# gercap/gr-ofdm_tools

Hardware: AMD Instinct MI355X
Metric: IQ Msamples/s Welch-PSD (4096-pt, 50% ovlp) (higher is better)
Workload: dtype f32; 1 GPU; C2: 2^28-sample complex64 stream, 4096-pt Hann Welch, 50% overlap, detrend constant, density; nfft=4096, noverlap=2048, window=hann, samples_per_gpu=268435456, segments_per_gpu=131071, parallelism=single GPU

## Files before the change

### gr-ofdm_tools_amd/csrc/abi_state.h

```cpp
#pragma once
#include "../../include/ofdm_tools_hip.h"
#include "oth_internal.h"
#include "abi_barrier.h"
#include "abi_mem.h"

#include <algorithm>
#include <cmath>
#include <cstdio>
#include <cstdlib>
#include <cstring>
#include <map>
#include <memory>
#include <mutex>
#include <new>
#include <string>
#include <vector>

using namespace oth;

struct oth_ctx {
    int device = 0;
    hipStream_t stream = nullptr;
    bool own_stream = false;
    int cu_count = 256;
    std::string err;
    std::string name;
    bool timing = false;
    std::vector<std::pair<Event, Event>> events;
    std::vector<std::pair<Event, Event>> free_events;
    double total_ms = 0.0;
    uint64_t launches = 0;
    std::map<int, DevBuf<float2>> twiddles;
    DevBuf<float> sink;
    DevBuf<double> acc4;
    DevBuf<unsigned> queue;
    unsigned *done_count = nullptr;
    std::recursive_mutex mu;
    bool queue_clean = false;
    int queue_used = 0;
    DevBuf<unsigned char> scratch;
    std::vector<int> bounds_host;
    DevBuf<int> d_bounds;
    PinnedBuf<int> h_bounds;
    Event bounds_ev;
    ~oth_ctx() {
        if (own_stream) hipStreamDestroy(stream);
    }
};

struct AnyTables {
    AnyShape sh{};
    const float2 *tw = nullptr;
    DevBuf<float2> chirp;
    DevBuf<float2> midtab;
    DevBuf<float2> ws;
    DevBuf<float4> mean;
};

struct oth_plan {
    oth_ctx *ctx = nullptr;
    int nfft = 0, nperseg = 0, noverlap = 0, step = 0, detrend = 0, scaling = 0, fftshift = 0, trim = 0;
    int db = 0, kernel = OTH_KERNEL_AUTO, sched = OTH_SCHED_DYNAMIC;
    double fs = 1.0, scale = 1.0;
    DevBuf<float> d_win;
    const float2 *d_tw = nullptr;
    DevBuf<float4> d_fd;
    DevBuf<float4> d_fd1x;
    DevBuf<float2> d_pilot;
    bool fast_detrend = false;
    bool rect_window = false;
    bool compl_window = false;
    DevBuf<float> d_partial;
    DevBuf<float> d_reduce;
    DevBuf<float> d_out;
    static constexpr int kOutRing = 4;
    PinnedBuf<float> h_out;
    PinnedBuf<unsigned> h_seq;
    uint64_t out_ticket[kOutRing] = {0, 0, 0, 0};
    uint64_t out_nseg[kOutRing] = {0, 0, 0, 0};
    uint64_t next_out_ticket = 1;
    bool pilot_launch = false;
    std::string last_recipe;
    DevBuf<float2> d_stage;
    DevBuf<float> d_sum;
    DevBuf<float> d_wpm;
    uint64_t nseg_total = 0;
    size_t carry = 0;
    DevBuf<float2> d_stream;
    std::string tune_variant;
    int tune_sched = -1, tune_chunk = 0, tune_tail = 0;
    PinnedBuf<char> h_ring[4];
    Event h_ring_ev[4];
    unsigned h_ring_next = 0;
    AnyTables any;
    std::mutex exec_mu;
    int hostwait = 0;
    int average = OTH_AVERAGE_MEAN;
    DevBuf<float> d_rows;
    DevBuf<float> d_med;
    DevBuf<unsigned> d_msel;
    AnyTables rows_any;
    long long bias_nseg = 0;
    double bias = 1.0;
    int ntapers = 0;
    DevBuf<float> d_tapers;
    DevBuf<float> d_coef;
};

struct oth_chain {
    oth_ctx *ctx = nullptr;
    int nfft = 0, fftshift = 0, epilogue = 0, keep_n = 1, count = 1;
    DevBuf<float> d_win;
    const float2 *d_tw = nullptr;
    DevBuf<float2> d_buf;
    size_t leftover = 0;
    DevBuf<float> d_rows;
    int do_iir = 0, do_peak = 0;
    float alpha = 0.f, kdb = 0.f;
    DevBuf<float> d_iir, d_peak;
// ... 182 lines not shown
```

### gr-ofdm_tools_amd/csrc/abi_welch.hip

```cpp
#include "abi_state.h"

#include <sched.h>
#include <time.h>

namespace {
bool window_spectrum(const std::vector<float> &w, int n, int band, std::vector<double> &re, std::vector<double> &im) {
    re.assign(n, 0.0);
    im.assign(n, 0.0);
    double s2 = 0.0;
    for (int i = 0; i < n; ++i) {
        re[i] = (double)w[i];
        s2 += (double)w[i] * (double)w[i];
    }
    host_fft_pow2(re, im);
    for (int k = band; k < n - band; ++k)
        if (re[k] * re[k] + im[k] * im[k] > 1e-10 * s2) return false;
    return true;
}

bool window_spectrum_table(const std::vector<float> &w, std::vector<float> &fd) {
    std::vector<double> re, im;
    if (!window_spectrum(w, 4096, 256, re, im)) return false;
    fd.resize(4 * 256);
    for (int t = 0; t < 256; ++t) {
// ... 5 lines not shown
    }
    return true;
}

bool window_spectrum_table_seg(const std::vector<float> &w, int n, std::vector<float> &fd) {
    const int R = n / 256, Q = 16 / R;
    std::vector<double> re, im;
    if (!window_spectrum(w, n, 256, re, im)) return false;
    fd.assign((size_t)4 * (n / 16) * Q, 0.f);
    for (int t = 0; t < n / 16; ++t) {
        const int k0 = t / R, j = t % R;
        for (int m = 0; m < Q; ++m) {
            const int lo = k0 + 16 * (j + R * m), hi = lo + 256 * (R - 1);
            float *o = &fd[4 * ((size_t)Q * t + m)];
            o[0] = (float)re[lo];
            o[1] = (float)im[lo];
            o[2] = (float)re[hi];
            o[3] = (float)im[hi];
        }
    }
    return true;
}

bool window_spectrum_table_16k(const std::vector<float> &w, int n, std::vector<float> &fd) {
    const int F = n / 4096;
    std::vector<double> re, im;
    if (!window_spectrum(w, n, 256 * F, re, im)) return false;
    fd.assign((size_t)4 * 256 * F, 0.f);
    for (int tid = 0; tid < 256 * F; ++tid) {
        const int kp = tid >> 8, k0 = (tid >> 4) & 15, k1 = tid & 15;
        const int lo = kp + F * (k0 + 16 * k1), hi = kp + F * (k0 + 16 * k1 + 3840);
        fd[4 * tid] = (float)re[lo];
        fd[4 * tid + 1] = (float)im[lo];
        fd[4 * tid + 2] = (float)re[hi];
        fd[4 * tid + 3] = (float)im[hi];
    }
    return true;
}

bool window_spectrum_table_1x(const std::vector<float> &w, int n, std::vector<float> &fd) {
    std::vector<double> re, im;
    if (!window_spectrum(w, n, 16, re, im)) return false;
    fd.assign((size_t)4 * (n / 16), 0.f);
    for (int k0 = 0; k0 < 16; ++k0) {
        const int lo = n == 16384 ? 64 * k0 : 64 * (k0 >> 1) + 32 * (k0 & 1);
        const int hi = n == 16384 ? 64 * k0 + 63 : 64 * (k0 >> 1) + 32 * (k0 & 1) + 31;
        fd[4 * lo] = (float)re[k0];
        fd[4 * lo + 1] = (float)im[k0];
        const int kh = n - 16 + k0;
        fd[4 * hi + 2] = (float)(-im[kh]);
        fd[4 * hi + 3] = (float)re[kh];
    }
    return true;
}

bool window_is_complementary(const std::vector<float> &w, int n) {
    for (int i = 0; i < n / 2; ++i)
        if (!(std::fabs((double)w[i] + (double)w[i + n / 2] - 1.0) <= 1.1920928955078125e-07)) return false;
    return true;
}

int segments(const oth_plan *p, size_t nsamples, long long *nseg) {
    if (nsamples < (size_t)p->nperseg) return OTH_ERR_INVALID;
    *nseg = (long long)((nsamples - (size_t)p->noverlap) / (size_t)p->step);
    return OTH_OK;
}

int run_average(oth_plan *p, const float2 *x, const float2 *y, size_t nsamples, int nstreams, size_t stride,
                long long *nseg_out, int *W_out, int *layout_out) {
    oth_ctx *c = p->ctx;
    long long nseg = 0;
    if (segments(p, nsamples, &nseg) != OTH_OK)
        return fail(c, OTH_ERR_INVALID, "input shorter than nperseg");
    const bool csd = (y != nullptr);
    if (p->ntapers) {
        if (csd) return refuse_mtm(p, "the cross spectrum", "the taper loop holds one channel");
        if (int rc = mtm_run(p, x, nseg, nstreams, stride, W_out)) return rc;
        *nseg_out = nseg;
        *layout_out = 0;
        return OTH_OK;
    }
    LaunchRecipe r;
    const char *why = "";
    if (int rrc = resolve_recipe(shape_of(p), csd, nseg, nstreams, c->cu_count, runtime_bpc, &r, &why))
        return fail(c, rrc, why);
    p->last_recipe = recipe_text(r, p->nfft);
    int rc = p->d_partial.ensure(c, sizeof(float) * (size_t)nstreams * r.W * r.nch * p->nfft);
    {
        const int groups = std::max(kReduceGroups, finalize_row_groups(p->nfft, r.W, r.nch));
        if (!rc) rc = p->d_reduce.ensure(c, sizeof(float) * (size_t)nstreams * groups * r.nch * p->nfft);
    }
    if (rc) return rc;
    const float4 *fd_tab = r.form == 2 ? (r.use_fd1x ? p->d_fd1x.get() : p->d_fd.get()) : nullptr;
    const float2 *pilot = nullptr;
    if (r.pilot == 1) {
        rc = p->d_pilot.ensure(c, sizeof(float2) * 2 * kPilotProbes * (size_t)nstreams);
        if (rc) return rc;
        HIPCHK(c, launch_pilot_mean(x, csd ? y : nullptr, stride, p->nperseg, p->step, nseg, nstreams, p->d_pilot.get(), c->stream));
        pilot = p->d_pilot.get();
    }
    unsigned *queue = nullptr;
    if (r.tickets) {
        queue = c->queue.get();
        if (!c->queue_clean) HIPCHK(c, hipMemsetAsync(c->queue.get(), 0, sizeof(unsigned) * 64, c->stream));
        c->queue_clean = false;
        c->queue_used = nstreams;
// ... 18 lines not shown
                         1.0f, 0, p->tune_variant == "anycov");
            if (rc) return rc;
        }
    } else if (r.kern == RK_SEG || r.kern == RK_SEGWS || r.kern == RK_SEGPAD) {
        SegArgs g{};
        g.x = x;
        g.stream_stride = stride;
        g.nstreams = nstreams;
        g.win = p->d_win.get();
        g.tw = p->d_tw;
        g.first = 0;
        g.step = p->step;
        g.nseg = nseg;
        g.detrend = p->detrend;
        g.chain = 0;
        g.partial = p->d_partial.get();
        g.wg_per_stream = r.W;
        g.sched = r.sched;
        g.chunk = r.chunk;
        g.tail_chunk = r.tail_chunk;
        g.nbig = r.nbig;
        g.queue = queue;
        g.fd = fd_tab;
        g.pilot = pilot;
        Timed tm(c);
        switch (r.kern) {
            case RK_SEGPAD: HIPCHK(c, launch_seg_padded(p->nfft, p->nperseg, g, r.seg_kind, c->stream)); break;
            case RK_SEGWS: HIPCHK(c, launch_segws(p->nfft, g, r.seg_det, c->stream)); break;
            default: HIPCHK(c, launch_seg(p->nfft, g, r.seg_kind, r.seg_wps4, c->stream)); break;
        }
    } else {
        WelchArgs a;
        a.x = x;
        a.y = y;
        a.win = p->d_win.get();
        a.tw = p->d_tw;
        a.partial = p->d_partial.get();
        a.nseg = nseg;
        a.stream_stride = stride;
        a.nperseg = p->nperseg;
        a.step = p->step;
        a.detrend = p->detrend;
        a.wg_per_stream = r.W;
        a.nstreams = nstreams;
        a.sched = r.sched;
        a.chunk = r.chunk;
        a.tail_chunk = r.tail_chunk;
        a.nbig = r.nbig;
        a.queue = queue;
        a.fd = fd_tab;
        a.pilot = pilot;
        a.pilot_inline = r.pilot == 2 ? 1 : 0;
        a.compl_win = p->compl_window && p->tune_variant != "wsgen" ? 1 : 0;
        Timed tm(c);
        switch (r.kern) {
            case RK_W4096: HIPCHK(c, r.variant->launch(a, c->stream)); break;
            case RK_CSD4096WS: HIPCHK(c, launch_csd_tuned4096ws(a, c->stream)); break;
            case RK_CSD4096: HIPCHK(c, launch_csd_tuned4096(a, c->stream)); break;
            case RK_W16K1X_HALF:
                HIPCHK(c, r.half_ws ? launch_welch_tuned8kws(a, c->stream) : launch_welch_tuned16k1x_half(p->nfft, a, c->stream));
                break;
            case RK_W16K1X: HIPCHK(c, launch_welch_tuned16k1x(p->nfft, a, r.x1_window, r.x1_plain, c->stream)); break;
            case RK_W16K: HIPCHK(c, launch_welch_tuned16k(p->nfft, a, c->stream)); break;
            default: HIPCHK(c, launch_welch_generic(p->nfft, a, c->stream)); break;
        }
    }
    *nseg_out = nseg;
    *W_out = r.W;
    *layout_out = r.layout;
    return OTH_OK;
}

int finalize_and_rearm(oth_ctx *c, FinalizeArgs &f, int nstreams) {
    f.queue_reset = nullptr;
    f.queue_n = 0;
    if (!c->queue_clean && c->queue_used > 0) {
        f.queue_reset = c->queue.get();
        f.queue_n = c->queue_used;
    }
    HIPCHK(c, launch_finalize(f, nstreams, c->stream));
    if (f.queue_reset) {
        c->queue_clean = true;
        c->queue_used = 0;
    }
    return OTH_OK;
}

FinalizeArgs finalize_args(const oth_plan *p, int W, int layout, int nch) {
    FinalizeArgs f{};
    f.partial = p->d_partial.get();
    f.scratch = p->d_reduce.get();
    f.W = W;
    f.nfft = p->nfft;
    f.nch = nch;
    f.layout = layout;
    f.l1 = p->any.sh.L1, f.l2 = p->any.sh.L2;
    return f;
}

double median_bias(long long n) {
    double b = 1.0;
    for (long long i = 1; i <= (n - 1) / 2; ++i) b += 1.0 / (double)(2 * i + 1) - 1.0 / (double)(2 * i);
    return b;
}

int refuse_median(oth_plan *p, const char *what) {
// ... 96 lines not shown
    if (use_device(c)) return OTH_ERR_HIP;
    std::unique_ptr<oth_plan> p(new (std::nothrow) oth_plan());
    if (!p) return fail(c, OTH_ERR_NOMEM, "host allocation failed");
    p->ctx = c;
    p->nfft = nfft;
    p->nperseg = nperseg;
    p->noverlap = noverlap;
    p->step = nperseg - noverlap;
    p->fast_detrend = detrend == OTH_DETREND_CONSTANT_FAST;
    p->detrend = detrend != OTH_DETREND_NONE ? OTH_DETREND_CONSTANT : OTH_DETREND_NONE;
    p->scaling = scaling;
    p->fs = fs;
    p->fftshift = fftshift != 0;
    p->trim = trim_bins;
    if (const char *e = getenv("OTH_HOSTWAIT")) p->hostwait = !strcmp(e, "sync") ? 1 : 0;
    *out = std::move(p);
    return OTH_OK;
}
}

extern "C" {

int oth_welch_plan(oth_ctx *c, int nfft, int nperseg, int noverlap, const float *window, int detrend, int scaling,
                   double fs, int fftshift, int trim_bins, oth_plan **out) {
    OTH_TRY
    CtxGuard guard_(c);
    if (!c || !out) return fail(c, OTH_ERR_INVALID, "ctx/out is NULL");
    *out = nullptr;
    std::unique_ptr<oth_plan> p;
    if (int rc = plan_begin(c, nfft, nperseg, noverlap, detrend, scaling, fs, fftshift, trim_bins, &p)) return rc;
    const bool any_route = !generic_supported(nfft);
    const bool det = p->detrend == OTH_DETREND_CONSTANT;
    if (const char *e = getenv("OTH_W4096_VARIANT")) p->tune_variant = e;
    if (const char *e = getenv("OTH_W4096_SCHED")) p->tune_sched = atoi(e);
    if (const char *e = getenv("OTH_W4096_CHUNK")) p->tune_chunk = atoi(e);
    if (const char *e = getenv("OTH_W4096_TAIL")) p->tune_tail = atoi(e);
    if (const char *e = getenv("OTH_PILOT_LAUNCH")) p->pilot_launch = atoi(e) != 0;
    std::vector<float> w(nfft, 0.f);
    double s1 = 0.0, s2 = 0.0;
    p->rect_window = true;
    for (int i = 0; i < nperseg; ++i) {
        w[i] = window ? window[i] : 1.0f;
        if (w[i] != 1.0f) p->rect_window = false;
        s1 += (double)w[i];
        s2 += (double)w[i] * (double)w[i];
    }
    switch (scaling) {
        case OTH_SCALE_DENSITY: p->scale = 1.0 / (fs * s2); break;
        case OTH_SCALE_OVER_N2: p->scale = 1.0 / ((double)nfft * (double)nfft); break;
        case OTH_SCALE_SPECTRUM: p->scale = 1.0 / (s1 * s1); break;
        default: p->scale = 1.0;
    }
    p->compl_window = nfft == 4096 && nperseg == 4096 && window_is_complementary(w, nfft);
    std::vector<float> fd, fd1x, wpm;
    const bool have_fd = det && ((nfft == 4096 && nperseg == 4096 && window_spectrum_table(w, fd)) ||
                                 (nfft == 2048 && nperseg == 2048 && window_spectrum_table_seg(w, nfft, fd)) ||
                                 ((nfft == 8192 || nfft == 16384) && nperseg == nfft && window_spectrum_table_16k(w, nfft, fd)));
    const bool have_fd1x = det && (nfft == 16384 || nfft == 8192) && nperseg == nfft && window_spectrum_table_1x(w, nfft, fd1x);
    if (any_route && nfft == 65536 && nperseg == 65536) {
        wpm.resize(65536);
        for (int n = 0; n < 32768; ++n) {
            wpm[n] = (float)((double)w[n] + (double)w[n + 32768]);
            wpm[32768 + n] = (float)((double)w[n] - (double)w[n + 32768]);
        }
    }
    if (int rc = any_route ? any_tables_init(c, nfft, &p->any) : get_twiddles(c, nfft, &p->d_tw)) return rc;
    hipError_t e = p->d_win.upload(c, w.data(), sizeof(float) * nfft);
    if (e == hipSuccess) e = p->d_sum.alloc(sizeof(float) * nfft);
    if (e == hipSuccess) e = hipMemsetAsync(p->d_sum.get(), 0, sizeof(float) * nfft, c->stream);
    if (e == hipSuccess && have_fd) e = p->d_fd.upload(c, fd.data(), sizeof(float) * fd.size());
    if (e == hipSuccess && have_fd1x) e = p->d_fd1x.upload(c, fd1x.data(), sizeof(float) * fd1x.size());
    if (e == hipSuccess && !wpm.empty()) e = p->d_wpm.upload(c, wpm.data(), sizeof(float) * wpm.size());
    const hipError_t es = hipStreamSynchronize(c->stream);
    if (e == hipSuccess) e = es;
    if (e != hipSuccess) return fail(c, OTH_ERR_HIP, std::string("plan setup: ") + hipGetErrorString(e));
    *out = p.release();
    return OTH_OK;
    OTH_CATCH(c)
}

int oth_plan_destroy(oth_plan *p) {
    OTH_TRY
    CtxGuard guard_(p ? p->ctx : nullptr);
    if (!p) return OTH_OK;
    oth_ctx *c = p->ctx;
    hipSetDevice(c->device);
    hipStreamSynchronize(c->stream);
    delete p;
    return OTH_OK;
    OTH_CATCH((p ? p->ctx : nullptr))
}

int oth_plan_set_output_db(oth_plan *p, int enable) {
    OTH_TRY
    CtxGuard guard_(p ? p->ctx : nullptr);
    if (!p) return fail(nullptr, OTH_ERR_INVALID, "plan is NULL");
    p->db = enable != 0;
    return OTH_OK;
    OTH_CATCH((p ? p->ctx : nullptr))
}

int oth_plan_set_kernel(oth_plan *p, int which) {
    OTH_TRY
    CtxGuard guard_(p ? p->ctx : nullptr);
    if (!p) return fail(nullptr, OTH_ERR_INVALID, "plan is NULL");
    if (which < OTH_KERNEL_AUTO || which > OTH_KERNEL_TUNED) return fail(p->ctx, OTH_ERR_INVALID, "unknown kernel id");
    if (p->ntapers && which == OTH_KERNEL_TUNED) return refuse_mtm(p, "OTH_KERNEL_TUNED", "no tuned kernel carries the taper loop");
    p->kernel = which;
    return OTH_OK;
    OTH_CATCH((p ? p->ctx : nullptr))
}

int oth_plan_set_schedule(oth_plan *p, int which) {
    OTH_TRY
    CtxGuard guard_(p ? p->ctx : nullptr);
    if (!p) return fail(nullptr, OTH_ERR_INVALID, "plan is NULL");
    if (which < OTH_SCHED_CONTIGUOUS || which > OTH_SCHED_DYNAMIC) return fail(p->ctx, OTH_ERR_INVALID, "unknown schedule");
    p->sched = which;
    return OTH_OK;
    OTH_CATCH((p ? p->ctx : nullptr))
}

int oth_plan_set_tuning(oth_plan *p, const char *variant, int sched, int chunk, int tail_chunk) {
// ... 567 lines not shown
```

### gr-ofdm_tools_amd/csrc/fft4096.hip.h

```cpp
#pragma once
#include "fft_lds.hip.h"
#include "oth_internal.h"

static_assert(oth::kPilotProbes == 8, "load_pilot() (fft_lds.hip.h) adds eight probe means");

namespace oth {
namespace {

constexpr int T4 = 256;
constexpr int RS = 272;
constexpr int LDS_X = 16 * RS;
constexpr int LDS_RED = 16;
constexpr size_t LDS_BYTES = (LDS_X + LDS_RED) * sizeof(float2);

constexpr float C1 = 0.92387953251128674f;
constexpr float S1 = 0.38268343236508977f;
constexpr float RH = 0.70710678118654752f;

__device__ __forceinline__ float2 mul_w1(float2 a) { return make_float2(fmaf(a.x, C1, a.y * S1), fmaf(a.y, C1, -a.x * S1)); }
__device__ __forceinline__ float2 mul_w2(float2 a) { return make_float2((a.x + a.y) * RH, (a.y - a.x) * RH); }
__device__ __forceinline__ float2 mul_w3(float2 a) { return make_float2(fmaf(a.x, S1, a.y * C1), fmaf(a.y, S1, -a.x * C1)); }
__device__ __forceinline__ float2 mul_w4(float2 a) { return make_float2(a.y, -a.x); }
__device__ __forceinline__ float2 mul_w6(float2 a) { return make_float2((a.y - a.x) * RH, -(a.x + a.y) * RH); }
__device__ __forceinline__ float2 mul_w9(float2 a) { return make_float2(-fmaf(a.x, C1, a.y * S1), fmaf(a.x, S1, -a.y * C1)); }
// ... 75 lines not shown
        v[1] = cadd(e1, o1);
        v[5] = csub(e1, o1);
        v[2] = cadd(e2, o2);
        v[6] = csub(e2, o2);
        v[3] = cadd(e3, o3);
        v[7] = csub(e3, o3);
        return;
    }
    const float2 p1 = make_float2(v[3].x + v[3].y, v[3].y - v[3].x);
    const float2 p3 = make_float2(v[7].y - v[7].x, -v[7].x - v[7].y);
    v[0] = cadd(e0, o0);
    v[4] = csub(e0, o0);
    v[1] = make_float2(fmaf(RH, p1.x, e1.x), fmaf(RH, p1.y, e1.y));
    v[5] = make_float2(fmaf(-RH, p1.x, e1.x), fmaf(-RH, p1.y, e1.y));
    v[2] = cadd(e2, o2);
    v[6] = csub(e2, o2);
    v[3] = make_float2(fmaf(RH, p3.x, e3.x), fmaf(RH, p3.y, e3.y));
    v[7] = make_float2(fmaf(-RH, p3.x, e3.x), fmaf(-RH, p3.y, e3.y));
}

template <int STRIDE, class F, class M>
__device__ __forceinline__ void dft16_from_lds(float2 (&v)[16], const float2 *base, F issued, M mid) {
    const unsigned addr = (unsigned)(unsigned long long)base;
    double r[16];
#define OTH_LDS_READ(i) asm volatile("ds_read_b64 %0, %1 offset:%2" : "=v"(r[i]) : "v"(addr), "n"(8 * STRIDE * (i)))
    OTH_LDS_READ(0); OTH_LDS_READ(4); OTH_LDS_READ(8); OTH_LDS_READ(12);
    OTH_LDS_READ(1); OTH_LDS_READ(5); OTH_LDS_READ(9); OTH_LDS_READ(13);
    OTH_LDS_READ(2); OTH_LDS_READ(6); OTH_LDS_READ(10); OTH_LDS_READ(14);
    OTH_LDS_READ(3); OTH_LDS_READ(7); OTH_LDS_READ(11); OTH_LDS_READ(15);
#undef OTH_LDS_READ
    issued();
#define OTH_LDS_WAIT(n, a, dep) \
    asm volatile("s_waitcnt lgkmcnt(" #n ")" : "+v"(r[a]), "+v"(r[a + 4]), "+v"(r[a + 8]), "+v"(r[a + 12]), "+v"(dep))
    float dep = 0.f;
#pragma unroll
    for (int a0 = 0; a0 < 4; ++a0) {
        if (a0 == 0) OTH_LDS_WAIT(12, 0, dep);
        else if (a0 == 1) OTH_LDS_WAIT(8, 1, v[0].x);
        else if (a0 == 2) OTH_LDS_WAIT(4, 2, v[1].x);
        else OTH_LDS_WAIT(0, 3, v[2].x);
#pragma unroll
        for (int j = 0; j < 4; ++j) v[a0 + 4 * j] = __builtin_bit_cast(float2, r[a0 + 4 * j]);
        dft4<false>(v[a0], v[a0 + 4], v[a0 + 8], v[a0 + 12]);
    }
#undef OTH_LDS_WAIT
    mid();
    dft16_layer2(v);
}
template <int STRIDE, class F>
__device__ __forceinline__ void dft16_from_lds(float2 (&v)[16], const float2 *base, F issued) {
    dft16_from_lds<STRIDE>(v, base, issued, [] {});
}

__device__ __forceinline__ float2 load_once(const float2 *p) {
    typedef float f2 __attribute__((ext_vector_type(2)));
    const f2 r = __builtin_nontemporal_load(reinterpret_cast<const f2 *>(p));
    return make_float2(r.x, r.y);
}

__device__ __forceinline__ void load_win(float &dst, unsigned lane_off, const char *row) {
    asm volatile("global_load_dword %0, %1, %2" : "=v"(dst) : "v"(lane_off), "s"(row) : "memory");
}

__device__ __forceinline__ long long chunk_count(const WelchArgs &p) {
    const long long rest = p.nseg - p.nbig * p.chunk;
    return p.nbig + (rest + p.tail_chunk - 1) / p.tail_chunk;
}
__device__ __forceinline__ void chunk_range(const WelchArgs &p, long long c, long long &sb, long long &se) {
    if (c < p.nbig) {
        sb = c * p.chunk;
        se = sb + p.chunk;
    } else {
        sb = p.nbig * p.chunk + (c - p.nbig) * p.tail_chunk;
        se = sb + p.tail_chunk < p.nseg ? sb + p.tail_chunk : p.nseg;
    }
}

template <class I> __device__ __forceinline__ I chunk_count_of(I nseg, I nbig, int chunk, int tail_chunk) {
    const I rest = nseg - nbig * chunk;
    return nbig + (rest + tail_chunk - 1) / tail_chunk;
}
template <class I> __device__ __forceinline__ void chunk_range_of(I nseg, I nbig, int chunk, int tail_chunk, I c, I &sb, I &se) {
    if (c < nbig) {
        sb = c * chunk;
        se = sb + chunk;
    } else {
        sb = nbig * chunk + (c - nbig) * tail_chunk;
        se = sb + tail_chunk < nseg ? sb + tail_chunk : nseg;
    }
}

__device__ __forceinline__ void prio_latency() { __builtin_amdgcn_s_setprio(2); }
__device__ __forceinline__ void prio_compute() { __builtin_amdgcn_s_setprio(0); }

__device__ __forceinline__ void lds_barrier() { asm volatile("s_waitcnt lgkmcnt(0)\n\ts_barrier" ::: "memory"); }

template <int STRIDE>
__device__ __forceinline__ void scatter_pow16(const float2 (&v)[16], float2 *out, float2 p1, float2 p4) {
    float2 wj[4], wi[4];
    wj[1] = p1;
    wi[1] = p4;
    asm volatile("" : "+v"(wj[1].x), "+v"(wj[1].y), "+v"(wi[1].x), "+v"(wi[1].y));
    wj[2] = cmul(wj[1], wj[1]);
    wj[3] = cmul(wj[2], wj[1]);
    wi[2] = cmul(wi[1], wi[1]);
    wi[3] = cmul(wi[2], wi[1]);
// ... 111 lines not shown
```

### gr-ofdm_tools_amd/csrc/oth_internal.h

```cpp
#pragma once
#include <hip/hip_runtime.h>
#include <stdint.h>
#include <stddef.h>

namespace oth {

constexpr int kPilotProbes = 8;

struct WelchArgs {
    const float2 *x;
    const float2 *y;
    const float *win;
    const float2 *tw;
    float *partial;
    long long nseg;
    size_t stream_stride;
    int nperseg;
    int step;
    int detrend;
    int wg_per_stream;
    int nstreams;
    int sched;
    int chunk;
    int tail_chunk;
    long long nbig;
    unsigned *queue;
    const float4 *fd;
    const float2 *pilot;
    int pilot_inline;
    int compl_win;
};

struct SegArgs {
    const float2 *x;
    size_t stream_stride;
    int nstreams;
    const float *win;
    const float2 *tw;
    const float4 *fd;
    const float2 *pilot;
    long long first;
    long long step;
    long long nseg;
    int detrend;
    int chain;
    float *partial;
    int acc_mode;
    long long acc_end;
    float l2;
    float *rows;
    long long store_from;
    int epilogue;
    float scale;
    int fftshift;
    int wg_per_stream;
    int sched;
    int chunk;
    int tail_chunk;
    long long nbig;
    unsigned *queue;
};

struct PgramArgs {
    const float2 *x;
    const float *win;
    const float2 *tw;
    float *rows;
    long long first_vec;
    long long nrows;
    int keep_n;
    int fftshift;
    int epilogue;
    float scale;
};

constexpr int kReduceGroups = 16;
inline int finalize_row_groups(int nfft, int W, int nch) {
    if (nch != 1 || nfft > 1024 || (nfft % 256) != 0 || W < 1024) return 0;
    return 65536 / nfft;
}

struct FinalizeArgs {
    const float *partial;
// ... 229 lines not shown
```

### gr-ofdm_tools_amd/csrc/welch4096ws.hip

```cpp

#include <type_traits>
#include "fft4096.hip.h"

namespace oth {
namespace {

constexpr int TWS = 512;
constexpr int WS_RED = 32;
constexpr int WS_CTRL = 16;
constexpr size_t WS_WIN_BYTES = 256 * 2 * sizeof(float4);
constexpr size_t WS_LDS_BYTES = (2 * LDS_X + WS_RED) * sizeof(float2) + WS_CTRL * sizeof(int) + WS_WIN_BYTES;

constexpr int WS_PAL = 2, WS_PAC = 0, WS_PAS = WS_PAL, WS_PBL = 2;
constexpr int WS_PBC = 1;

enum { ITEM_STOP = 0, ITEM_DATA = 1, ITEM_BUBBLE = 2 };

#ifndef OTH_WS_COMPL_POWERS
#define OTH_WS_COMPL_POWERS 13
#endif
constexpr int WS_COMPL_POWERS = OTH_WS_COMPL_POWERS;

template <bool DETREND, bool PILOT, bool COMPL>
__device__ __forceinline__ void welch4096ws_body(const WelchArgs &p) {
    static_assert(DETREND || !PILOT, "the pilot belongs to the detrend");
    extern __shared__ __attribute__((aligned(16))) unsigned char smem[];
    float2 *img = reinterpret_cast<float2 *>(smem);
    float2 *red = img + 2 * LDS_X;
    int *ctrl = reinterpret_cast<int *>(red + WS_RED);

    const int tid = threadIdx.x;
    const bool producer = tid < 256;
    const int t = tid & 255;
    const int hi = t >> 4, lo = t & 15;
    const int wave = t >> 6;
    const int wg = blockIdx.x, W = p.wg_per_stream, stream = blockIdx.y;
    const float2 *xb = p.x + (size_t)stream * p.stream_stride;
    const int sched = p.sched;
    const long long nchunks = sched ? chunk_count(p) : 1;

    const int w1 = hi * 17 + lo, r1 = hi * RS + lo, w2 = hi * RS + lo, r2 = hi * RS + lo * 17;

    if (producer) {
        float win[COMPL ? 1 : 8];
        float4 *wl = reinterpret_cast<float4 *>(ctrl + WS_CTRL) + t;
        constexpr int WROW = COMPL ? 0 : 8;
        if constexpr (!COMPL) {
#pragma unroll
            for (int a = 0; a < 8; ++a) win[a] = p.win[256 * a + t];
        }
        wl[0] = make_float4(p.win[256 * WROW + t], p.win[256 * (WROW + 1) + t], p.win[256 * (WROW + 2) + t], p.win[256 * (WROW + 3) + t]);
        wl[256] = make_float4(p.win[256 * (WROW + 4) + t], p.win[256 * (WROW + 5) + t], p.win[256 * (WROW + 6) + t],
                              p.win[256 * (WROW + 7) + t]);
        const float2 b1 = p.tw[t], b2 = p.tw[2 * t], b3 = p.tw[3 * t], b4 = p.tw[4 * t], b8 = p.tw[8 * t],
                     b12 = p.tw[(12 * t) & 4095];
        float2 bm[WS_COMPL_POWERS - 6 > 0 && COMPL ? WS_COMPL_POWERS - 6 : 1];
        if constexpr (COMPL) {
#pragma unroll
            for (int k = 0; k < WS_COMPL_POWERS - 6; ++k) bm[k] = p.tw[((5 + k + k / 3) * t) & 4095];
        }
        float2 kw[8], nxt[8];
        float2 prev_new = make_float2(0.f, 0.f);
        float2 pv = make_float2(0.f, 0.f);
        if (PILOT && !p.pilot_inline) pv = load_pilot(p.pilot, stream);
        int it = 0;
        unsigned ticket = 0;
        using std::false_type;
        using std::true_type;
        using mid = std::integral_constant<int, 0>;
        using head = std::integral_constant<int, 1>;
        using none = std::integral_constant<int, 2>;

        auto uni = [](int v) { return __builtin_amdgcn_readfirstlane(v); };
// ... 100 lines not shown
            }
            sb = uni((int)((p.nseg * wg) / W));
            se = uni((int)((p.nseg * (wg + 1)) / W));
            return sb < se;
        };
        bool have = open_chunk(sched ? wg : 0);
        if (have) load_chunk_head(sb);
        if (PILOT && p.pilot_inline) {
            const bool own = sched == 0 && have;
            const PilotProbes probes = inline_pilot_load(own ? xb + (size_t)sb * 2048 : xb, own ? (long long)(se - sb) : p.nseg, 2048, t);
            inline_pilot_store(probes, t, img + LDS_X);
            lds_barrier();
            pv = inline_pilot_value(img + LDS_X);
        }
        while (have) {
            const int n = se - sb;
            int ncur = 0;
            if (n >= 2) {
                item(true_type{}, mid{}, sb, 0, n == 2);
                int s = sb + 1;
                if (s < se - 1) item(false_type{}, mid{}, s++, 0, true);
                for (; s + 1 < se - 1; s += 2) {
                    item(false_type{}, mid{}, s, 0, false);
                    item(false_type{}, mid{}, s + 1, 0, false);
                }
                if (s < se - 1) item(false_type{}, mid{}, s, 0, false);
                ncur = (sched == 1) ? cur + W : W + uni(ctrl[4]);
                int nsb = 0, nse = 0;
                const bool have_next = sched && ncur < nchunks;
                if (have_next) {
                    range(ncur, nsb, nse);
                    item(false_type{}, head{}, se - 1, nsb, false);
                    cur = ncur;
                    sb = nsb;
                    se = nse;
                    continue;
                }
                item(false_type{}, none{}, se - 1, 0, false);
                break;
            }
            item(true_type{}, none{}, sb, 0, true);
            if (sched == 0) break;
            if (sched == 2) {
                step_end(ITEM_BUBBLE);
                ncur = W + uni(ctrl[4]);
            } else {
                ncur = cur + W;
            }
            have = open_chunk(ncur);
            if (have) load_chunk_head(sb);
        }
        step_end(ITEM_STOP);
    } else {
        float2 tw2[16];
#pragma unroll
        for (int k = 1; k < 16; ++k) tw2[k] = p.tw[16 * lo * k];
        float4 fw = make_float4(0.f, 0.f, 0.f, 0.f);
        if (DETREND) fw = p.fd[t];
        float acc[16];
#pragma unroll
        for (int k = 0; k < 16; ++k) acc[k] = 0.f;
        float2 v[16];
        float2 mean = make_float2(0.f, 0.f);
        asm volatile("s_waitcnt vmcnt(0)"
                     : "+v"(tw2[1].x), "+v"(tw2[1].y), "+v"(tw2[2].x), "+v"(tw2[2].y), "+v"(tw2[3].x), "+v"(tw2[3].y), "+v"(tw2[4].x),
                       "+v"(tw2[4].y), "+v"(tw2[5].x), "+v"(tw2[5].y), "+v"(tw2[6].x), "+v"(tw2[6].y), "+v"(tw2[7].x), "+v"(tw2[7].y));
        asm volatile("" : "+v"(tw2[8].x), "+v"(tw2[8].y), "+v"(tw2[9].x), "+v"(tw2[9].y), "+v"(tw2[10].x), "+v"(tw2[10].y),
                          "+v"(tw2[11].x), "+v"(tw2[11].y), "+v"(tw2[12].x), "+v"(tw2[12].y), "+v"(tw2[13].x), "+v"(tw2[13].y));
        asm volatile("" : "+v"(tw2[14].x), "+v"(tw2[14].y), "+v"(tw2[15].x), "+v"(tw2[15].y), "+v"(fw.x), "+v"(fw.y), "+v"(fw.z),
                          "+v"(fw.w));
        int it = 0;
        auto next_item = [&]() -> int {
            __builtin_amdgcn_s_setprio(WS_PBL);
            lds_barrier();
            const int q = it & 1;
            const float2 *lq = img + q * LDS_X;
            const int kind = ctrl[q];
            const float2 h0 = red[q * 8], h1 = red[q * 8 + 1], h2 = red[q * 8 + 2], h3 = red[q * 8 + 3];
            dft16_from_lds<17>(v, lq + r1, [] { __builtin_amdgcn_s_setprio(WS_PBC); });
            if (DETREND) {
                const float2 tot = cadd(cadd(h0, h1), cadd(h2, h3));
                mean = make_float2(tot.x * (1.0f / 4096.0f), tot.y * (1.0f / 4096.0f));
            }
            ++it;
            return kind;
        };
        if (PILOT && p.pilot_inline) lds_barrier();
        int item = next_item();
        for (;;) {
            while (item == ITEM_BUBBLE) item = next_item();
            if (item == ITEM_STOP) break;
            float2 *lx = img + ((it & 1) ^ 1) * LDS_X;
            __builtin_amdgcn_s_setprio(WS_PBL);
            lx[w2] = v[r16(0)];
#pragma unroll
            for (int k1 = 1; k1 < 16; ++k1) lx[w2 + k1 * 17] = cmul(v[r16(k1)], tw2[k1]);
            wave_lds_sync();
            dft16_from_lds<1>(v, lx + r2, [] { __builtin_amdgcn_s_setprio(WS_PBC); });
            if (DETREND) {
                v[r16(0)] = make_float2(v[r16(0)].x - (mean.x * fw.x - mean.y * fw.y),
                                        v[r16(0)].y - (mean.x * fw.y + mean.y * fw.x));
                v[r16(15)] = make_float2(v[r16(15)].x - (mean.x * fw.z - mean.y * fw.w),
                                         v[r16(15)].y - (mean.x * fw.w + mean.y * fw.z));
            }
#pragma unroll
            for (int k2 = 0; k2 < 16; ++k2) {
                const float2 X = v[r16(k2)];
                acc[k2] = fmaf(X.x, X.x, fmaf(X.y, X.y, acc[k2]));
            }
            item = next_item();
        }
        float *dst = p.partial + ((size_t)stream * W + wg) * 4096;
#pragma unroll
        for (int k2 = 0; k2 < 16; ++k2) dst[256 * k2 + t] = acc[k2];
    }
}

template <bool DETREND, bool PILOT = false>
__global__ __launch_bounds__(TWS, 4) void welch4096ws_kernel(WelchArgs p) {
    welch4096ws_body<DETREND, PILOT, false>(p);
}
template <bool DETREND, bool PILOT = false>
__global__ __launch_bounds__(TWS, 4) void welch4096ws_compl_kernel(WelchArgs p) {
    welch4096ws_body<DETREND, PILOT, true>(p);
}

}

int tuned4096_blocks_per_cu_ws() {
    static int cached = 0;
    if (cached) return cached;
    int n = 0;
    if (hipOccupancyMaxActiveBlocksPerMultiprocessor(&n, welch4096ws_kernel<true, false>, TWS, WS_LDS_BYTES) != hipSuccess || n < 1)
        n = 1;
    return cached = n;
}

hipError_t launch_welch_tuned4096_ws(const WelchArgs &a, hipStream_t s) {
    const dim3 grid(a.wg_per_stream, a.nstreams);
    static bool armed[64] = {};
    int dev = 0;
    if (hipGetDevice(&dev) != hipSuccess || dev < 0 || dev >= 64) dev = 63, armed[63] = false;
    bool &big_lds = armed[dev];
    if (!big_lds) {
        hipError_t e = hipSuccess;
        for (const void *fn : {reinterpret_cast<const void *>(welch4096ws_kernel<true, true>),
                               reinterpret_cast<const void *>(welch4096ws_kernel<true, false>),
                               reinterpret_cast<const void *>(welch4096ws_kernel<false, false>),
                               reinterpret_cast<const void *>(welch4096ws_compl_kernel<true, true>),
                               reinterpret_cast<const void *>(welch4096ws_compl_kernel<true, false>),
                               reinterpret_cast<const void *>(welch4096ws_compl_kernel<false, false>)})
            if (e == hipSuccess) e = hipFuncSetAttribute(fn, hipFuncAttributeMaxDynamicSharedMemorySize, (int)WS_LDS_BYTES);
        if (e != hipSuccess) return e;
        big_lds = true;
    }
    const bool pilot = a.detrend && (a.pilot || a.pilot_inline);
    if (a.compl_win) {
        if (pilot) hipLaunchKernelGGL((welch4096ws_compl_kernel<true, true>), grid, dim3(TWS), WS_LDS_BYTES, s, a);
        else if (a.detrend) hipLaunchKernelGGL((welch4096ws_compl_kernel<true, false>), grid, dim3(TWS), WS_LDS_BYTES, s, a);
        else hipLaunchKernelGGL((welch4096ws_compl_kernel<false, false>), grid, dim3(TWS), WS_LDS_BYTES, s, a);
    } else if (pilot)
        hipLaunchKernelGGL((welch4096ws_kernel<true, true>), grid, dim3(TWS), WS_LDS_BYTES, s, a);
    else if (a.detrend)
        hipLaunchKernelGGL((welch4096ws_kernel<true, false>), grid, dim3(TWS), WS_LDS_BYTES, s, a);
    else
        hipLaunchKernelGGL((welch4096ws_kernel<false, false>), grid, dim3(TWS), WS_LDS_BYTES, s, a);
    return hipGetLastError();
}

}
```

Before: 455,600 Msamples/s.

## Use tangent-factored twiddles in 4096-pt Welch FFT second pass

Replaces the complex twiddle multiplies between the two radix-16 passes with tangent-form multiplies (one FMA per component), deferring the cosine factors into a scaled radix-16 DFT whose constants come from a per-thread precomputed table. The goal is to cut VALU work in the FFT inner loop of the work-stealing 4096 kernel. It adds 33 per-thread table registers (more VGPR pressure) and a host-side table build, and tan-based factoring can lose accuracy near small cosines, which the code handles by clamping.

```diff
diff --git a/gr-ofdm_tools_amd/csrc/abi_state.h b/gr-ofdm_tools_amd/csrc/abi_state.h
--- a/gr-ofdm_tools_amd/csrc/abi_state.h
+++ b/gr-ofdm_tools_amd/csrc/abi_state.h
@@ -65,6 +65,7 @@
     DevBuf<float> d_win;
     const float2 *d_tw = nullptr;
     DevBuf<float4> d_fd;
+    DevBuf<float> d_tantw;
     DevBuf<float4> d_fd1x;
     DevBuf<float2> d_pilot;
     bool fast_detrend = false;
diff --git a/gr-ofdm_tools_amd/csrc/abi_welch.hip b/gr-ofdm_tools_amd/csrc/abi_welch.hip
--- a/gr-ofdm_tools_amd/csrc/abi_welch.hip
+++ b/gr-ofdm_tools_amd/csrc/abi_welch.hip
@@ -81,6 +81,34 @@
         fd[4 * hi + 3] = (float)re[kh];
     }
     return true;
+}
+
+void tangent_twiddle_table(std::vector<float> &tab) {
+    const double kClamp = 1.0 / 1073741824.0, c1 = std::cos(M_PI / 8.0), rh = std::sqrt(0.5);
+    auto split = [&](int m, double &c, double &t) {
+        const double a = -2.0 * M_PI * (double)(m & 255) / 256.0;
+        c = std::cos(a);
+        if (std::fabs(c) < kClamp) c = kClamp;
+        t = std::sin(a) / c;
+    };
+    tab.assign((size_t)kTanRows * 256, 0.f);
+    for (int t = 0; t < 256; ++t) {
+        const int lo = t & 15;
+        double s[16], K[18], tn;
+        for (int k = 1; k < 16; ++k) {
+            split(lo * k, s[0], tn);
+            tab[256 * (kTanEx2 + k - 1) + t] = (float)tn;
+        }
+        for (int c = 0; c < 16; ++c) split(lo * c, s[c], tn);
+        for (int a = 0; a < 4; ++a) {
+            K[3 * a] = s[a + 8] / s[a];
+            K[3 * a + 1] = s[a + 12] / s[a + 4];
+            K[3 * a + 2] = s[a + 4] / s[a];
+        }
+        K[12] = s[2] / s[0], K[13] = s[3] / s[1], K[14] = s[1] / s[0];
+        K[15] = rh * K[12], K[16] = c1 * K[14], K[17] = rh * K[14];
+        for (int k = 0; k < 18; ++k) tab[256 * (kTanK3 + k) + t] = (float)K[k];
+    }
 }
 
 bool window_is_complementary(const std::vector<float> &w, int n) {
@@ -205,6 +233,7 @@
         a.pilot = pilot;
         a.pilot_inline = r.pilot == 2 ? 1 : 0;
         a.compl_win = p->compl_window && p->tune_variant != "wsgen" ? 1 : 0;
+        a.tantw = p->d_tantw.get();
         Timed tm(c);
         switch (r.kern) {
             case RK_W4096: HIPCHK(c, r.variant->launch(a, c->stream)); break;
@@ -407,7 +436,8 @@
         default: p->scale = 1.0;
     }
     p->compl_window = nfft == 4096 && nperseg == 4096 && window_is_complementary(w, nfft);
-    std::vector<float> fd, fd1x, wpm;
+    std::vector<float> fd, fd1x, wpm, tantw;
+    if (nfft == 4096 && nperseg == 4096) tangent_twiddle_table(tantw);
     const bool have_fd = det && ((nfft == 4096 && nperseg == 4096 && window_spectrum_table(w, fd)) ||
                                  (nfft == 2048 && nperseg == 2048 && window_spectrum_table_seg(w, nfft, fd)) ||
                                  ((nfft == 8192 || nfft == 16384) && nperseg == nfft && window_spectrum_table_16k(w, nfft, fd)));
@@ -424,6 +454,7 @@
     if (e == hipSuccess) e = p->d_sum.alloc(sizeof(float) * nfft);
     if (e == hipSuccess) e = hipMemsetAsync(p->d_sum.get(), 0, sizeof(float) * nfft, c->stream);
     if (e == hipSuccess && have_fd) e = p->d_fd.upload(c, fd.data(), sizeof(float) * fd.size());
+    if (e == hipSuccess && !tantw.empty()) e = p->d_tantw.upload(c, tantw.data(), sizeof(float) * tantw.size());
     if (e == hipSuccess && have_fd1x) e = p->d_fd1x.upload(c, fd1x.data(), sizeof(float) * fd1x.size());
     if (e == hipSuccess && !wpm.empty()) e = p->d_wpm.upload(c, wpm.data(), sizeof(float) * wpm.size());
     const hipError_t es = hipStreamSynchronize(c->stream);
diff --git a/gr-ofdm_tools_amd/csrc/fft4096.hip.h b/gr-ofdm_tools_amd/csrc/fft4096.hip.h
--- a/gr-ofdm_tools_amd/csrc/fft4096.hip.h
+++ b/gr-ofdm_tools_amd/csrc/fft4096.hip.h
@@ -151,6 +151,84 @@
     dft16_from_lds<STRIDE>(v, base, issued, [] {});
 }
 
+__device__ __forceinline__ void dft4_tail_qr(float2 t0, float2 t1, float2 q, float2 r, float S, float2 &a0, float2 &a1, float2 &a2,
+                                             float2 &a3) {
+    a0 = make_float2(fmaf(S, q.x, t0.x), fmaf(S, q.y, t0.y));
+    a2 = make_float2(fmaf(-S, q.x, t0.x), fmaf(-S, q.y, t0.y));
+    a1 = make_float2(fmaf(S, r.y, t1.x), fmaf(-S, r.x, t1.y));
+    a3 = make_float2(fmaf(-S, r.y, t1.x), fmaf(S, r.x, t1.y));
+}
+__device__ __forceinline__ void dft4_scaled(float2 &a0, float2 &a1, float2 &a2, float2 &a3, float r2, float r31, float k) {
+    const float2 t0 = make_float2(fmaf(r2, a2.x, a0.x), fmaf(r2, a2.y, a0.y));
+    const float2 t1 = make_float2(fmaf(-r2, a2.x, a0.x), fmaf(-r2, a2.y, a0.y));
+    const float2 q = make_float2(fmaf(r31, a3.x, a1.x), fmaf(r31, a3.y, a1.y));
+    const float2 r = make_float2(fmaf(-r31, a3.x, a1.x), fmaf(-r31, a3.y, a1.y));
+    dft4_tail_qr(t0, t1, q, r, k, a0, a1, a2, a3);
+}
+__device__ __forceinline__ void dft16_layer2_scaled(float2 (&v)[16], const float (&K)[18]) {
+    const float G2 = K[12], G31 = K[13], G1 = K[14], RHG2 = K[15], C1G1 = K[16], RHG1 = K[17];
+    dft4_scaled(v[0], v[1], v[2], v[3], G2, G31, G1);
+    {
+        const float2 u1 = v[5], u2 = v[6], u3 = v[7];
+        const float2 p1 = make_float2(fmaf(T1, u1.y, u1.x), fmaf(-T1, u1.x, u1.y));
+        const float2 p2 = make_float2(u2.x + u2.y, u2.y - u2.x);
+        const float2 p3 = make_float2(fmaf(T1, u3.x, u3.y), fmaf(T1, u3.y, -u3.x));
+        const float2 t0 = make_float2(fmaf(RHG2, p2.x, v[4].x), fmaf(RHG2, p2.y, v[4].y));
+        const float2 t1 = make_float2(fmaf(-RHG2, p2.x, v[4].x), fmaf(-RHG2, p2.y, v[4].y));
+        const float2 q = make_float2(fmaf(G31, p3.x, p1.x), fmaf(G31, p3.y, p1.y));
+        const float2 r = make_float2(fmaf(-G31, p3.x, p1.x), fmaf(-G31, p3.y, p1.y));
+        dft4_tail_qr(t0, t1, q, r, C1G1, v[4], v[5], v[6], v[7]);
+    }
+    {
+        const float2 u1 = v[9], u2 = v[10], u3 = v[11];
+        const float2 p1 = make_float2(u1.x + u1.y, u1.y - u1.x);
+        const float2 p3 = make_float2(u3.y - u3.x, -u3.x - u3.y);
+        const float2 t0 = make_float2(fmaf(G2, u2.y, v[8].x), fmaf(-G2, u2.x, v[8].y));
+        const float2 t1 = make_float2(fmaf(-G2, u2.y, v[8].x), fmaf(G2, u2.x, v[8].y));
+        const float2 q = make_float2(fmaf(G31, p3.x, p1.x), fmaf(G31, p3.y, p1.y));
+        const float2 r = make_float2(fmaf(-G31, p3.x, p1.x), fmaf(-G31, p3.y, p1.y));
+        dft4_tail_qr(t0, t1, q, r, RHG1, v[8], v[9], v[10], v[11]);
+    }
+    {
+        const float2 u1 = v[13], u2 = v[14], u3 = v[15];
+        const float2 p1 = make_float2(fmaf(T1, u1.x, u1.y), fmaf(T1, u1.y, -u1.x));
+        const float2 p2 = make_float2(u2.y - u2.x, -u2.x - u2.y);
+        const float2 p3 = make_float2(fmaf(-T1, u3.y, -u3.x), fmaf(T1, u3.x, -u3.y));
+        const float2 t0 = make_float2(fmaf(RHG2, p2.x, v[12].x), fmaf(RHG2, p2.y, v[12].y));
+        const float2 t1 = make_float2(fmaf(-RHG2, p2.x, v[12].x), fmaf(-RHG2, p2.y, v[12].y));
+        const float2 q = make_float2(fmaf(G31, p3.x, p1.x), fmaf(G31, p3.y, p1.y));
+        const float2 r = make_float2(fmaf(-G31, p3.x, p1.x), fmaf(-G31, p3.y, p1.y));
+        dft4_tail_qr(t0, t1, q, r, C1G1, v[12], v[13], v[14], v[15]);
+    }
+}
+template <int STRIDE, class F>
+__device__ __forceinline__ void dft16_scaled_from_lds(float2 (&v)[16], const float2 *base, const float (&K)[18], F issued) {
+    const unsigned addr = (unsigned)(unsigned long long)base;
+    double r[16];
+#define OTH_LDS_READ(i) asm volatile("ds_read_b64 %0, %1 offset:%2" : "=v"(r[i]) : "v"(addr), "n"(8 * STRIDE * (i)))
+    OTH_LDS_READ(0); OTH_LDS_READ(4); OTH_LDS_READ(8); OTH_LDS_READ(12);
+    OTH_LDS_READ(1); OTH_LDS_READ(5); OTH_LDS_READ(9); OTH_LDS_READ(13);
+    OTH_LDS_READ(2); OTH_LDS_READ(6); OTH_LDS_READ(10); OTH_LDS_READ(14);
+    OTH_LDS_READ(3); OTH_LDS_READ(7); OTH_LDS_READ(11); OTH_LDS_READ(15);
+#undef OTH_LDS_READ
+    issued();
+#define OTH_LDS_WAIT(n, a, dep) \
+    asm volatile("s_waitcnt lgkmcnt(" #n ")" : "+v"(r[a]), "+v"(r[a + 4]), "+v"(r[a + 8]), "+v"(r[a + 12]), "+v"(dep))
+    float dep = 0.f;
+#pragma unroll
+    for (int a0 = 0; a0 < 4; ++a0) {
+        if (a0 == 0) OTH_LDS_WAIT(12, 0, dep);
+        else if (a0 == 1) OTH_LDS_WAIT(8, 1, v[0].x);
+        else if (a0 == 2) OTH_LDS_WAIT(4, 2, v[1].x);
+        else OTH_LDS_WAIT(0, 3, v[2].x);
+#pragma unroll
+        for (int j = 0; j < 4; ++j) v[a0 + 4 * j] = __builtin_bit_cast(float2, r[a0 + 4 * j]);
+        dft4_scaled(v[a0], v[a0 + 4], v[a0 + 8], v[a0 + 12], K[3 * a0], K[3 * a0 + 1], K[3 * a0 + 2]);
+    }
+#undef OTH_LDS_WAIT
+    dft16_layer2_scaled(v, K);
+}
+
 __device__ __forceinline__ float2 load_once(const float2 *p) {
     typedef float f2 __attribute__((ext_vector_type(2)));
     const f2 r = __builtin_nontemporal_load(reinterpret_cast<const f2 *>(p));
diff --git a/gr-ofdm_tools_amd/csrc/oth_internal.h b/gr-ofdm_tools_amd/csrc/oth_internal.h
--- a/gr-ofdm_tools_amd/csrc/oth_internal.h
+++ b/gr-ofdm_tools_amd/csrc/oth_internal.h
@@ -6,6 +6,10 @@
 namespace oth {
 
 constexpr int kPilotProbes = 8;
+
+constexpr int kTanEx2 = 0;
+constexpr int kTanK3 = 15;
+constexpr int kTanRows = 33;
 
 struct WelchArgs {
     const float2 *x;
@@ -29,6 +33,7 @@
     const float2 *pilot;
     int pilot_inline;
     int compl_win;
+    const float *tantw;
 };
 
 struct SegArgs {
diff --git a/gr-ofdm_tools_amd/csrc/welch4096ws.hip b/gr-ofdm_tools_amd/csrc/welch4096ws.hip
--- a/gr-ofdm_tools_amd/csrc/welch4096ws.hip
+++ b/gr-ofdm_tools_amd/csrc/welch4096ws.hip
@@ -19,6 +19,11 @@
 #ifndef OTH_WS_COMPL_POWERS
 #define OTH_WS_COMPL_POWERS 13
 #endif
+#ifndef OTH_WS_PLAIN_TW
+#define OTH_WS_PLAIN_TW 0
+#endif
+constexpr bool WS_TANTW = !OTH_WS_PLAIN_TW;
+
 constexpr int WS_COMPL_POWERS = OTH_WS_COMPL_POWERS;
 
 template <bool DETREND, bool PILOT, bool COMPL>
@@ -225,9 +230,17 @@
         }
         step_end(ITEM_STOP);
     } else {
-        float2 tw2[16];
-#pragma unroll
-        for (int k = 1; k < 16; ++k) tw2[k] = p.tw[16 * lo * k];
+        float2 tw2[WS_TANTW ? 1 : 16];
+        float tt[WS_TANTW ? 16 : 1], K3[18];
+        if constexpr (WS_TANTW) {
+#pragma unroll
+            for (int k = 1; k < 16; ++k) tt[k] = p.tantw[256 * (kTanEx2 + k - 1) + t];
+#pragma unroll
+            for (int k = 0; k < 18; ++k) K3[k] = p.tantw[256 * (kTanK3 + k) + t];
+        } else {
+#pragma unroll
+            for (int k = 1; k < 16; ++k) tw2[k] = p.tw[16 * lo * k];
+        }
         float4 fw = make_float4(0.f, 0.f, 0.f, 0.f);
         if (DETREND) fw = p.fd[t];
         float acc[16];
@@ -235,13 +248,16 @@
         for (int k = 0; k < 16; ++k) acc[k] = 0.f;
         float2 v[16];
         float2 mean = make_float2(0.f, 0.f);
-        asm volatile("s_waitcnt vmcnt(0)"
-                     : "+v"(tw2[1].x), "+v"(tw2[1].y), "+v"(tw2[2].x), "+v"(tw2[2].y), "+v"(tw2[3].x), "+v"(tw2[3].y), "+v"(tw2[4].x),
-                       "+v"(tw2[4].y), "+v"(tw2[5].x), "+v"(tw2[5].y), "+v"(tw2[6].x), "+v"(tw2[6].y), "+v"(tw2[7].x), "+v"(tw2[7].y));
-        asm volatile("" : "+v"(tw2[8].x), "+v"(tw2[8].y), "+v"(tw2[9].x), "+v"(tw2[9].y), "+v"(tw2[10].x), "+v"(tw2[10].y),
-                          "+v"(tw2[11].x), "+v"(tw2[11].y), "+v"(tw2[12].x), "+v"(tw2[12].y), "+v"(tw2[13].x), "+v"(tw2[13].y));
-        asm volatile("" : "+v"(tw2[14].x), "+v"(tw2[14].y), "+v"(tw2[15].x), "+v"(tw2[15].y), "+v"(fw.x), "+v"(fw.y), "+v"(fw.z),
-                          "+v"(fw.w));
+        asm volatile("s_waitcnt vmcnt(0)" : "+v"(fw.x), "+v"(fw.y), "+v"(fw.z), "+v"(fw.w));
+        if constexpr (WS_TANTW) {
+#pragma unroll
+            for (int k = 1; k < 16; ++k) asm volatile("" : "+v"(tt[k]));
+#pragma unroll
+            for (int k = 0; k < 18; ++k) asm volatile("" : "+v"(K3[k]));
+        } else {
+#pragma unroll
+            for (int k = 1; k < 16; ++k) asm volatile("" : "+v"(tw2[k].x), "+v"(tw2[k].y));
+        }
         int it = 0;
         auto next_item = [&]() -> int {
             __builtin_amdgcn_s_setprio(WS_PBL);
@@ -267,9 +283,14 @@
             __builtin_amdgcn_s_setprio(WS_PBL);
             lx[w2] = v[r16(0)];
 #pragma unroll
-            for (int k1 = 1; k1 < 16; ++k1) lx[w2 + k1 * 17] = cmul(v[r16(k1)], tw2[k1]);
+            for (int k1 = 1; k1 < 16; ++k1) {
+                const float2 u = v[r16(k1)];
+                if constexpr (WS_TANTW) lx[w2 + k1 * 17] = make_float2(fmaf(-tt[k1], u.y, u.x), fmaf(tt[k1], u.x, u.y));
+                else lx[w2 + k1 * 17] = cmul(u, tw2[k1]);
+            }
             wave_lds_sync();
-            dft16_from_lds<1>(v, lx + r2, [] { __builtin_amdgcn_s_setprio(WS_PBC); });
+            if constexpr (WS_TANTW) dft16_scaled_from_lds<1>(v, lx + r2, K3, [] { __builtin_amdgcn_s_setprio(WS_PBC); });
+            else dft16_from_lds<1>(v, lx + r2, [] { __builtin_amdgcn_s_setprio(WS_PBC); });
             if (DETREND) {
                 v[r16(0)] = make_float2(v[r16(0)].x - (mean.x * fw.x - mean.y * fw.y),
                                         v[r16(0)].y - (mean.x * fw.y + mean.y * fw.x));
@@ -311,6 +332,7 @@
 
 hipError_t launch_welch_tuned4096_ws(const WelchArgs &a, hipStream_t s) {
     const dim3 grid(a.wg_per_stream, a.nstreams);
+    if (WS_TANTW && !a.tantw) return hipErrorInvalidValue;
     static bool armed[64] = {};
     int dev = 0;
     if (hipGetDevice(&dev) != hipSuccess || dev < 0 || dev >= 64) dev = 63, armed[63] = false;
```

Result: slower. 444,700 Msamples/s (-2.4%).
